# vicpc00/td-vc-gan

Measured on AMD Instinct MI355X. Metric: audio-seconds/sec (G+D train step, stage-1), higher is better.
Workload: dtype f32 (fp32 storage and accumulation everywhere; FiLM cond_var.2 forward and weight-grad as split-bf16 x6 products -- three exact bf16 pieces per operand, six piece products on the bf16 MFMA, fp32 accumulate: fp32-level accuracy; every other kernel exact-fp32 MFMA)

## Files before the change

td-vc-gan_amd/csrc/conv_api.hip:

```cpp
#include "../../include/tdvc.h"
#include "conv_common.h"
#include "conv_lean.h"
#include "conv_wgrad_lean.h"
#include "conv_small_group.h"
#include "api_util.h"

namespace tdvc {
template <int MODE> hipError_t launch_conv_gemm(GemmConvP, int, hipStream_t);
template <int MODE> hipError_t launch_conv_scalar(GemmConvP, int, hipStream_t);
template <int MODE> hipError_t launch_conv_wgrad(WgradP, int, int, hipStream_t);
template <int MODE> hipError_t launch_conv_wgrad_scalar(WgradP, int, long, float*, hipStream_t);
int wgrad_geometry(WgradP& p, int B, int* bpb_out);
bool wgrad_mfma_supported(int J);
hipError_t launch_slab_reduce(const float*, int, long, long, float*, int, long, hipStream_t, long n_w = -1, float* dbias = nullptr);
hipError_t launch_bias_grad(const Opnd&, int, int, int, float*, hipStream_t);
hipError_t fold_flush(hipStream_t st);
void fold_set_defer(int on);
void fold_reset(hipStream_t st);
}

namespace tdvc {


}

using namespace tdvc;

static inline bool al16(const void* p) { return (((uintptr_t)p) & 15) == 0; }
static inline bool ok_bs(const void* p, long bs) { return !p || (bs < (1L << 31)); }
static inline bool vec_ptr(const void* p, long bs) { return !p || (al16(p) && (bs & 3) == 0); }

static int lean_xfk(const tdvc_xform& x, float* slope, float* scale, const float** aux, long* aux_bs) {
  *scale = x.scale == 0.f ? 1.f : x.scale; *aux = x.aux; *aux_bs = x.aux_bs; *slope = x.slope;
  switch (x.kind) {
    case TDVC_XF_NONE: *slope = 1.f; *aux = nullptr; return LXF_ACT;
    case TDVC_XF_LRELU: *aux = nullptr; return (x.slope >= 0.f && x.slope <= 1.f) ? LXF_ACT : -1;
    case TDVC_XF_FILM_LRELU: return (x.slope >= 0.f && x.slope <= 1.f) ? LXF_FILM : -1;
    case TDVC_XF_MASK_LRELU: return LXF_MASK_LRELU;
    case TDVC_XF_MASK_TANH: return LXF_MASK_TANH;
    default: return -1;
  }
}

static bool lean_shape_ok(const tdvc_conv_desc* d) {
  return d->kind == TDVC_CONV && d->stride == 1 && d->groups == 1 && d->Tin == d->Tout && ((d->Tin & 3) == 0 || d->Tin <= 80);
}

namespace tdvc { int g_force_generic = 0; }
extern "C" void tdvc_set_force_generic(int on) { g_force_generic = on; }

static Xf to_xf(const tdvc_xform& x) {
  Xf r; r.kind = x.kind; r.slope = x.slope; r.scale = x.scale == 0.f ? 1.f : x.scale;
  r.aux = x.aux; r.aux_bs = x.aux_bs; return r;
}

static int check_desc(const tdvc_conv_desc* d) {
  if (!d) return tdvc_fail(TDVC_EINVAL, "null desc");
  if (d->B <= 0 || d->Cin <= 0 || d->Cout <= 0 || d->Tin <= 0 || d->Tout <= 0 || d->K <= 0 || d->stride <= 0 ||
      d->dilation <= 0 || d->groups <= 0 || d->pad < 0)
    return tdvc_fail(TDVC_EINVAL, "conv desc: non-positive dimension");
  if (d->Cin % d->groups || d->Cout % d->groups) return tdvc_fail(TDVC_EINVAL, "conv desc: channels not divisible by groups");
  if (d->stride > 1 && d->dilation != 1) return tdvc_fail(TDVC_EUNSUPPORTED, "strided conv with dilation");
  if (d->reflect && (d->stride != 1 || d->kind != TDVC_CONV)) return tdvc_fail(TDVC_EUNSUPPORTED, "reflect padding needs stride 1 conv");
  if (d->reflect && d->pad >= d->Tin) return tdvc_fail(TDVC_EINVAL, "reflect padding must be smaller than the input length");
  if (d->w_cin < 0 || d->w_cin_off < 0) return tdvc_fail(TDVC_EINVAL, "conv desc: negative weight channel window");
  if (d->w_cin > 0) {
    if (d->groups != 1 || d->kind != TDVC_CONV) return tdvc_fail(TDVC_EUNSUPPORTED, "weight channel window needs a plain conv with groups == 1");
    if (d->w_cin_off + d->Cin > d->w_cin) return tdvc_fail(TDVC_EINVAL, "conv desc: weight channel window out of range");
  }
  if (d->kind == TDVC_CONV) {
    long expect = ((long)d->Tin + 2L * d->pad - (long)d->dilation * (d->K - 1) - 1) / d->stride + 1;
    if (expect != d->Tout) return tdvc_fail(TDVC_EINVAL, "conv desc: Tout does not match conv arithmetic");
  } else if (d->kind == TDVC_CONV_TRANSPOSE) {
    if (d->stride < 2) return tdvc_fail(TDVC_EUNSUPPORTED, "transposed conv needs stride >= 2");
    long expect = ((long)d->Tin - 1) * d->stride - 2L * d->pad + (d->K - 1) + 1;
    if (d->Tout > expect + d->stride - 1 || d->Tout < expect) return tdvc_fail(TDVC_EINVAL, "conv desc: Tout does not match transposed conv arithmetic");
  } else return tdvc_fail(TDVC_EINVAL, "conv desc: unknown kind");
  return TDVC_OK;
}

static inline int ceil_div(int a, int b) { return (a + b - 1) / b; }

static bool small_group_ok(const tdvc_conv_desc* d) {
  return !g_force_generic && g_knob[2] == 0 && d->kind == TDVC_CONV && d->groups >= 16 && d->Cin == 4 * d->groups && d->Cout == 4 * d->groups &&
         d->dilation == 1 && !d->reflect && d->w_cin == 0 && d->stride >= 2 && d->stride <= 8 && d->K <= 48;
}
static void small_group_base(const tdvc_conv_desc* d, SmallGroupP& q) {
  q.B = d->B; q.G = d->groups; q.Tin = d->Tin; q.Tout = d->Tout; q.K = d->K; q.s = d->stride; q.pad = d->pad;
  q.in_scale = 1.f; q.out_scale = 1.f; q.dy_scale = 1.f;
}

static bool use_mfma(const GemmConvP& p) {
  if (g_force_generic) return false;
  if (p.R <= 2 && p.x.Cg == 1 && p.Cy_g <= 2) return false;
  return (long)p.Cred * p.J >= 7;
}

template <int MODE>
static int run_gemm(GemmConvP& p, int B, hipStream_t st) {
  hipError_t e = use_mfma(p) ? launch_conv_gemm<MODE>(p, B, st) : launch_conv_scalar<MODE>(p, B, st);
  return e == hipSuccess ? TDVC_OK : tdvc_fail(TDVC_ELAUNCH, hipGetErrorString(e));
}

static int dispatch_gemm(GemmConvP& p, int B, hipStream_t st) {
  switch (p.mode) {
    case MODE_DIRECT: return run_gemm<MODE_DIRECT>(p, B, st);
    case MODE_DOWN: return run_gemm<MODE_DOWN>(p, B, st);
    default: return run_gemm<MODE_UP>(p, B, st);
  }
}

extern "C" int tdvc_conv_fwd(const tdvc_conv_desc* d, const tdvc_conv_fwd_args* a, void* stream) {
  if (int rc = check_desc(d)) return rc;
  if (!a || !a->x || !a->w || !a->y) return tdvc_fail(TDVC_EINVAL, "conv_fwd: null pointer");
  const int Cin_g = d->Cin / d->groups, Cout_g = d->Cout / d->groups;
  if (small_group_ok(d) && a->x_xf.kind <= TDVC_XF_LRELU && !a->res && !a->add && !a->bias3) {
    SmallGroupP q = {};
    small_group_base(d, q);
    q.x = a->x; q.x_bs = a->x_bs; q.w = a->w; q.bias = a->bias; q.y = a->y; q.y_bs = a->y_bs;
    q.act_in = a->x_xf.kind == TDVC_XF_LRELU; q.slope_in = a->x_xf.slope; q.in_scale = a->x_xf.scale == 0.f ? 1.f : a->x_xf.scale;
    q.post = a->post_act; q.post_slope = a->post_slope; q.out_scale = a->out_scale == 0.f ? 1.f : a->out_scale;
    const hipError_t e = launch_small_group_fwd(q, (hipStream_t)stream);
    if (e == hipSuccess) return TDVC_OK;
    if (e != hipErrorNotSupported) return tdvc_fail(TDVC_ELAUNCH, hipGetErrorString(e));
  }
  if (!g_force_generic && lean_shape_ok(d) && (d->Cin & 3) == 0) {
    LeanP q = {};
    float slope, scale; const float* aux; long aux_bs;
    const int xfk = lean_xfk(a->x_xf, &slope, &scale, &aux, &aux_bs);
    const int cw = (d->w_cin > 0 ? d->w_cin : d->Cin) * d->K;
    const float* w = a->w + (long)d->w_cin_off * d->K;
    if (xfk >= 0 && (cw & 3) == 0 && al16(w) && ok_bs(a->x, a->x_bs) && ok_bs(a->y, a->y_bs) && ok_bs(a->res, a->res_bs) &&
        ok_bs(a->add, a->add_bs) && ok_bs(aux, aux_bs)) {
      q.x = a->x; q.w = w; q.y = a->y; q.bias = a->bias; q.bias3 = a->bias3; q.res = a->res; q.add = a->add; q.aux = aux;
      q.x_bs = (int)a->x_bs; q.y_bs = (int)a->y_bs; q.res_bs = (int)a->res_bs; q.add_bs = (int)a->add_bs; q.aux_bs = (int)aux_bs;
      q.T = d->Tin; q.Cin = d->Cin; q.Cout = d->Cout; q.Cw = cw; q.K = d->K; q.d = d->dilation; q.pad = d->pad; q.reflect = d->reflect;
      q.post = a->post_act; q.slope = slope; q.in_scale = scale; q.out_scale = a->out_scale == 0.f ? 1.f : a->out_scale;
      q.add_scale = 1.f; q.m_slope = a->post_slope;
      q.sbits = a->sign_bits; q.sb_bs = (int)a->sign_bits_bs;
      q.vec = ((d->Tin & 3) == 0 && vec_ptr(a->x, a->x_bs) && vec_ptr(a->y, a->y_bs) && vec_ptr(a->res, a->res_bs) &&
               vec_ptr(a->add, a->add_bs) && vec_ptr(aux, aux_bs)) ? 1 : 0;
      if (!q.vec && d->Tin > 80) goto generic_fwd;
      hipError_t e = launch_conv_lean(q, d->B, xfk, EPI_FWD, (hipStream_t)stream);
      if (e == hipSuccess) return TDVC_OK;
      if (e != hipErrorNotSupported) return tdvc_fail(TDVC_ELAUNCH, hipGetErrorString(e));
    }
  }
generic_fwd:
  if (a->sign_bits) return tdvc_fail(TDVC_EUNSUPPORTED, "conv_fwd: sign_bits needs a stride-1 conv with Tout % 32 == 0, Tout > 80 and 16-byte aligned operands");
  GemmConvP p = {};
  p.x.p = a->x; p.x.bs = a->x_bs; p.x.T = d->Tin; p.x.Cg = Cin_g; p.x.xf = to_xf(a->x_xf);
  p.w = a->w; p.K = d->K; p.s = d->stride; p.pad = d->pad; p.groups = d->groups;
  p.y = a->y; p.y_bs = a->y_bs; p.Ty = d->Tout; p.Cy_g = Cout_g;
  p.epi = EPI_FWD; p.bias = a->bias; p.bias3 = a->bias3; p.res = a->res; p.res_bs = a->res_bs;
  p.post = a->post_act; p.post_slope = a->post_slope; p.out_scale = a->out_scale == 0.f ? 1.f : a->out_scale;
  p.add = a->add; p.add_bs = a->add_bs; p.add_scale = 1.f;
  p.w_sg = (long)Cout_g * Cin_g * d->K;
  if (d->kind == TDVC_CONV) {
    p.w_sm = (long)Cin_g * d->K; p.w_sc = d->K;
    if (d->w_cin > 0) { p.w_sm = (long)d->w_cin * d->K; p.w += (long)d->w_cin_off * d->K; }
    p.R = Cout_g; p.N = d->Tout;
    if (d->stride == 1) { p.mode = MODE_DIRECT; p.Cred = Cin_g; p.J = d->K; p.d = d->dilation; p.reflect = d->reflect; }
    else { p.mode = MODE_DOWN; p.Cred = Cin_g * d->stride; p.J = ceil_div(d->K, d->stride); p.d = 1; }
  } else {
    p.w_sm = d->K; p.w_sc = (long)Cout_g * d->K;
    p.mode = MODE_UP; p.R = Cout_g * d->stride; p.Cred = Cin_g; p.J = ceil_div(d->K, d->stride); p.d = 1;
    p.N = (d->Tout - 1 + d->pad) / d->stride + 1;
  }
  return dispatch_gemm(p, d->B, (hipStream_t)stream);
}

extern "C" int tdvc_conv_dgrad(const tdvc_conv_desc* d, const tdvc_conv_dgrad_args* a, void* stream) {
  if (int rc = check_desc(d)) return rc;
  if (!a || !a->dy || !a->w || !a->dx) return tdvc_fail(TDVC_EINVAL, "conv_dgrad: null pointer");
  const int Cin_g = d->Cin / d->groups, Cout_g = d->Cout / d->groups;
  if (small_group_ok(d) && a->epilogue == TDVC_DG_PLAIN && !a->add &&
      (a->dy_xf.kind == TDVC_XF_NONE || (a->dy_xf.kind == TDVC_XF_MASK_LRELU && a->dy_xf.aux))) {
    SmallGroupP q = {};
    small_group_base(d, q);
    q.dy = a->dy; q.dy_bs = a->dy_bs; q.w = a->w; q.y = a->dx; q.y_bs = a->dx_bs;
    q.dy_scale = a->dy_xf.scale == 0.f ? 1.f : a->dy_xf.scale;
    if (a->dy_xf.kind == TDVC_XF_MASK_LRELU) { q.mask = a->dy_xf.aux; q.mask_bs = a->dy_xf.aux_bs; q.m_slope = a->dy_xf.slope; }
    const hipError_t e = launch_small_group_dgrad(q, (hipStream_t)stream);
    if (e == hipSuccess) return TDVC_OK;
    if (e != hipErrorNotSupported) return tdvc_fail(TDVC_ELAUNCH, hipGetErrorString(e));
  }
  if (!g_force_generic && a->wt && lean_shape_ok(d) && (d->Cout & 3) == 0 && (d->K - 1) * d->dilation - d->pad >= 0) {
    LeanP q = {};
    float slope, scale; const float* aux; long aux_bs;
    const int xfk = lean_xfk(a->dy_xf, &slope, &scale, &aux, &aux_bs);
    const int cw = d->Cout * d->K;
    const float* w = a->wt + (long)d->w_cin_off * cw;
    const int epi = a->epilogue == TDVC_DG_PLAIN ? EPI_PLAIN : (a->epilogue == TDVC_DG_MASK_LRELU ? EPI_MASK : EPI_FILM);
    if (xfk >= 0 && (cw & 3) == 0 && al16(w) && ok_bs(a->dy, a->dy_bs) && ok_bs(a->dx, a->dx_bs) && ok_bs(a->add, a->add_bs) &&
        ok_bs(aux, aux_bs) && ok_bs(a->x_in, a->x_in_bs) && ok_bs(a->gb, a->gb_bs) && ok_bs(a->dgb, a->dgb_bs) &&
        (epi == EPI_PLAIN || a->x_in || (epi == EPI_MASK && a->x_sign_bits)) && (epi != EPI_FILM || (a->gb && a->dgb))) {
      q.x = a->dy; q.w = w; q.y = a->dx; q.add = a->add; q.aux = aux; q.mx = a->x_in; q.gb = a->gb; q.dgb = a->dgb;
      q.x_bs = (int)a->dy_bs; q.y_bs = (int)a->dx_bs; q.add_bs = (int)a->add_bs; q.aux_bs = (int)aux_bs; q.mx_bs = (int)a->x_in_bs;
      q.gb_bs = (int)a->gb_bs; q.dgb_bs = (int)a->dgb_bs;
      q.T = d->Tin; q.Cin = d->Cout; q.Cout = d->Cin; q.Cw = cw; q.K = d->K; q.d = d->dilation;
      q.pad = (d->K - 1) * d->dilation - d->pad; q.flip = 1; q.mirror = d->reflect ? d->pad : 0;
      q.slope = slope; q.in_scale = scale; q.out_scale = 1.f; q.add_scale = a->add_scale; q.m_slope = a->slope;
      if (epi == EPI_MASK && a->x_sign_bits) { q.mbits = a->x_sign_bits; q.mb_bs = (int)a->x_sign_bits_bs; }
      q.vec = ((d->Tin & 3) == 0 && vec_ptr(a->dy, a->dy_bs) && vec_ptr(a->dx, a->dx_bs) && vec_ptr(a->add, a->add_bs) && vec_ptr(aux, aux_bs) &&
               vec_ptr(a->x_in, a->x_in_bs) && vec_ptr(a->gb, a->gb_bs) && vec_ptr(a->dgb, a->dgb_bs)) ? 1 : 0;
      if (!q.vec && d->Tin > 80) goto generic_dgrad;
      hipError_t e = launch_conv_lean(q, d->B, xfk, epi, (hipStream_t)stream);
      if (e == hipSuccess) return TDVC_OK;
      if (e != hipErrorNotSupported) return tdvc_fail(TDVC_ELAUNCH, hipGetErrorString(e));
      if (q.mbits && a->x_in) {
        q.mbits = nullptr;
        e = launch_conv_lean(q, d->B, xfk, epi, (hipStream_t)stream);
        if (e == hipSuccess) return TDVC_OK;
        if (e != hipErrorNotSupported) return tdvc_fail(TDVC_ELAUNCH, hipGetErrorString(e));
      }
    }
  }
generic_dgrad:
  if (a->epilogue == TDVC_DG_MASK_LRELU && !a->x_in && a->x_sign_bits)
    return tdvc_fail(TDVC_EUNSUPPORTED, "conv_dgrad: x_sign_bits without x_in needs a stride-1 conv with Tin % 32 == 0, Tin > 80 and 16-byte aligned operands");
  GemmConvP p = {};
  p.x.p = a->dy; p.x.bs = a->dy_bs; p.x.T = d->Tout; p.x.Cg = Cout_g; p.x.xf = to_xf(a->dy_xf);
  p.w = a->w; p.K = d->K; p.s = d->stride; p.groups = d->groups;
  p.y = a->dx; p.y_bs = a->dx_bs; p.Ty = d->Tin; p.Cy_g = Cin_g; p.N = d->Tin;
  p.add = a->add; p.add_bs = a->add_bs; p.add_scale = a->add_scale;
  p.w_sg = (long)Cout_g * Cin_g * d->K;
  switch (a->epilogue) {
    case TDVC_DG_PLAIN: p.epi = EPI_PLAIN; break;
    case TDVC_DG_MASK_LRELU:
      if (!a->x_in) return tdvc_fail(TDVC_EINVAL, "conv_dgrad: mask epilogue needs x_in");
      p.epi = EPI_MASK; p.mx = a->x_in; p.mx_bs = a->x_in_bs; p.m_slope = a->slope; break;
    case TDVC_DG_FILM:
      if (!a->x_in || !a->gb || !a->dgb) return tdvc_fail(TDVC_EINVAL, "conv_dgrad: FiLM epilogue needs x_in, gb, dgb");
      p.epi = EPI_FILM; p.mx = a->x_in; p.mx_bs = a->x_in_bs; p.m_slope = a->slope;
      p.gb = a->gb; p.gb_bs = a->gb_bs; p.dgb = a->dgb; p.dgb_bs = a->dgb_bs; break;
    default: return tdvc_fail(TDVC_EINVAL, "conv_dgrad: unknown epilogue");
  }
  if (d->kind == TDVC_CONV) {
    p.w_sm = d->K; p.w_sc = (long)Cin_g * d->K;
    if (d->w_cin > 0) { p.w_sc = (long)d->w_cin * d->K; p.w += (long)d->w_cin_off * d->K; }
    if (d->stride == 1) {
      p.mode = MODE_DIRECT; p.R = Cin_g; p.Cred = Cout_g; p.J = d->K; p.d = d->dilation; p.tap_flip = 1;
      p.pad = (d->K - 1) * d->dilation - d->pad;
      if (p.pad < 0) return tdvc_fail(TDVC_EUNSUPPORTED, "conv_dgrad: padding larger than the receptive field");
      p.mirror_pad = d->reflect ? d->pad : 0;
    } else {
      p.mode = MODE_UP; p.R = Cin_g * d->stride; p.Cred = Cout_g; p.J = ceil_div(d->K, d->stride); p.d = 1; p.pad = d->pad;
      p.N = (d->Tin - 1 + d->pad) / d->stride + 1;
    }
  } else {
    p.w_sm = (long)Cout_g * d->K; p.w_sc = d->K;
    p.mode = MODE_DOWN; p.R = Cin_g; p.Cred = Cout_g * d->stride; p.J = ceil_div(d->K, d->stride); p.d = 1; p.pad = d->pad;
  }
  return dispatch_gemm(p, d->B, (hipStream_t)stream);
}

static void fill_wgrad(const tdvc_conv_desc* d, const tdvc_conv_wgrad_args* a, WgradP& p) {
  const int Cin_g = d->Cin / d->groups, Cout_g = d->Cout / d->groups;
  p.groups = d->groups; p.K = d->K; p.s = d->stride; p.pad = d->pad;
  p.w_sg = (long)Cout_g * Cin_g * d->K;
  if (d->kind == TDVC_CONV) {
    if (a) { p.a.p = a->dy; p.a.bs = a->dy_bs; p.a.xf = to_xf(a->dy_xf); p.x.p = a->x; p.x.bs = a->x_bs; p.x.xf = to_xf(a->x_xf); }
    p.a.T = d->Tout; p.a.Cg = Cout_g; p.x.T = d->Tin; p.x.Cg = Cin_g;
    p.R = Cout_g; p.N = d->Tout; p.w_sm = (long)Cin_g * d->K; p.w_sc = d->K;
    if (d->stride == 1) { p.mode = MODE_DIRECT; p.Cred = Cin_g; p.J = d->K; p.d = d->dilation; p.reflect = d->reflect; }
    else { p.mode = MODE_DOWN; p.Cred = Cin_g * d->stride; p.J = ceil_div(d->K, d->stride); p.d = 1; }
  } else {
    if (a) { p.a.p = a->x; p.a.bs = a->x_bs; p.a.xf = to_xf(a->x_xf); p.x.p = a->dy; p.x.bs = a->dy_bs; p.x.xf = to_xf(a->dy_xf); }
    p.a.T = d->Tin; p.a.Cg = Cin_g; p.x.T = d->Tout; p.x.Cg = Cout_g;
    p.R = Cin_g; p.N = d->Tin; p.w_sm = (long)Cout_g * d->K; p.w_sc = d->K;
    p.mode = MODE_DOWN; p.Cred = Cout_g * d->stride; p.J = ceil_div(d->K, d->stride); p.d = 1;
  }
}

static bool wgrad_use_mfma(const WgradP& p) {
  if (g_force_generic) return false;
  if (p.R <= 2 && p.x.Cg == 1) return false;
  if (!wgrad_mfma_supported(p.J)) return false;
  return true;
}

static bool wgrad_lean_ok(const tdvc_conv_desc* d) {
  const bool wide = d->Cout >= 32 && d->Cin >= 32;
  return !g_force_generic && d->kind == TDVC_CONV && d->stride == 1 && d->groups == 1 && d->Tin == d->Tout &&
         (d->Tout > 128 || wide) && wgrad_lean_supported(d->K, d->dilation) && (d->K != 15 || d->Cout <= 16 || d->Cin <= 16);
}

namespace tdvc {
int wgrad_lean_nslab(int R, int Cin, int N, int K, int B);
bool wgrad_x6_ok(int R, int Cin, int T, int K, int dil, int pad, int reflect);
void wgrad_x6_plan(int R, int T, int B, int* ntiles, int* tpb, int* ngroups);
hipError_t launch_conv_wgrad_x6(const WgLeanP& q, int B, hipStream_t st);
}
static bool wgrad_x6_desc_ok(const tdvc_conv_desc* d) {
  return !g_force_generic && d->kind == TDVC_CONV && d->stride == 1 && d->groups == 1 && d->Tin == d->Tout && d->w_cin == 0 &&
         wgrad_x6_ok(d->Cout, d->Cin, d->Tout, d->K, d->dilation, d->pad, d->reflect);
}

extern "C" size_t tdvc_conv_wgrad_workspace(const tdvc_conv_desc* d) {
  if (check_desc(d)) return 0;
  size_t small = small_group_ok(d) ? small_group_wgrad_workspace(d->B, d->groups, d->K) : 0;
  if (wgrad_lean_ok(d)) {
    size_t lean = (size_t)wgrad_lean_nslab(d->Cout, d->Cin, d->Tout, d->K, d->B) * ((size_t)d->Cout * d->Cin * d->K + d->Cout) * sizeof(float);
    if (wgrad_x6_desc_ok(d)) {
      int nt, tpb, ng;
      wgrad_x6_plan(d->Cout, d->Tout, d->B, &nt, &tpb, &ng);
      const size_t x6 = (size_t)ng * ((size_t)d->Cout * d->Cin * d->K + d->Cout) * sizeof(float);
      if (x6 > lean) lean = x6;
    }
    return lean;
  }
  WgradP p = {};
  fill_wgrad(d, nullptr, p);
  if (!wgrad_use_mfma(p)) return small;
  int bpb;
  const int nslab = wgrad_geometry(p, d->B, &bpb);
  const long wsize = (long)d->groups * p.w_sg;
  const size_t gen = (size_t)nslab * (size_t)wsize * sizeof(float);
  return gen > small ? gen : small;
}

extern "C" int tdvc_conv_wgrad(const tdvc_conv_desc* d, const tdvc_conv_wgrad_args* a, void* stream) {
  if (int rc = check_desc(d)) return rc;
  if (!a || !a->x || !a->dy) return tdvc_fail(TDVC_EINVAL, "conv_wgrad: null pointer");
  hipStream_t st = (hipStream_t)stream;
  WgradP p = {};
  fill_wgrad(d, a, p);
  const long wsize = (long)d->groups * p.w_sg;
  hipError_t e = hipSuccess;
  bool done = false, bias_done = false;
  if (a->dw && small_group_ok(d) && a->x_xf.kind <= TDVC_XF_LRELU &&
      (a->dy_xf.kind == TDVC_XF_NONE || (a->dy_xf.kind == TDVC_XF_MASK_LRELU && a->dy_xf.aux))) {
    SmallGroupP q = {};
    small_group_base(d, q);
    q.x = a->x; q.x_bs = a->x_bs; q.dy = a->dy; q.dy_bs = a->dy_bs;
    q.act_in = a->x_xf.kind == TDVC_XF_LRELU; q.slope_in = a->x_xf.slope; q.in_scale = a->x_xf.scale == 0.f ? 1.f : a->x_xf.scale;
// ... 100 lines not shown
```

td-vc-gan_amd/csrc/conv_common.h:

```cpp
#pragma once
#include <hip/hip_runtime.h>
#include <stdint.h>
#include <mutex>

#define TDVC_BIG_LDS_ONCE(k)                                                                                         \
  do {                                                                                                               \
    static std::once_flag f_;                                                                                        \
    std::call_once(f_, [&] { hipFuncSetAttribute(reinterpret_cast<const void*>(k), hipFuncAttributeMaxDynamicSharedMemorySize, 160 * 1024); }); \
  } while (0)
namespace tdvc {
extern int g_trace_on;
extern int g_force_tile;
extern int g_force_generic;
extern int g_lds_cap;
extern int g_knob[8];
void trace_kernel(const void* fn);
}
#define TDVC_TRACE(k) do { if (tdvc::g_trace_on) tdvc::trace_kernel(reinterpret_cast<const void*>(k)); } while (0)

namespace tdvc {

enum { MODE_DIRECT = 0, MODE_DOWN = 1, MODE_UP = 2 };
enum { XF_NONE = 0, XF_LRELU = 1, XF_FILM_LRELU = 2, XF_MASK_LRELU = 3, XF_MASK_TANH = 4 };
enum { EPI_FWD = 0, EPI_MASK = 1, EPI_FILM = 2, EPI_PLAIN = 3 };
enum { POST_NONE = 0, POST_LRELU = 1, POST_TANH = 2 };

struct Xf {
  int kind; float slope; float scale;
  const float* aux; long aux_bs;
};

struct Opnd {
  const float* p; long bs; int T; int Cg; Xf xf;
};

struct GemmConvP {
  Opnd x;
  const float* w; long w_sg, w_sm, w_sc; int K; int tap_flip;
  int mode, s, d, pad, reflect, J;
  int R, Cred, Cc, N, groups, lo, span, XS, WS;
  int i0;
  int mirror_pad;
  int stage_rows;
  int chan_stage;
  int w_nat;
  int w_packed;
  float* y; long y_bs; int Ty; int Cy_g;
  int epi;
  const float* bias;
  const float* bias3;
  const float* res; long res_bs;
  int post; float post_slope; float out_scale;
  const float* add; long add_bs; float add_scale;
  const float* mx; long mx_bs; float m_slope;
  const float* gb; long gb_bs; float* dgb; long dgb_bs;
};

struct WgradP {
  Opnd a;
  Opnd x;
  int mode, s, d, pad, reflect, J, K;
  int R, Cred, N, groups, lo, span, NTc, XS, AS;
  int i0;
  int ntiles;
  float* slab; long slab_stride;
  long w_sg, w_sm, w_sc;
};

__device__ __forceinline__ float lrelu_f(float v, float s) { return v > 0.f ? v : v * s; }

__device__ __forceinline__ float apply_xf(const Xf& xf, float v, int b, int ch, int t, int T, int Ctot) {
  switch (xf.kind) {
    case XF_LRELU: v = lrelu_f(v, xf.slope); break;
    case XF_FILM_LRELU: {
      const float* g = xf.aux + (long)b * xf.aux_bs + (long)ch * T + t;
      v = lrelu_f(v * (1.f + g[0]) + g[(long)Ctot * T], xf.slope);
    } break;
    case XF_MASK_LRELU: {
      float a = xf.aux[(long)b * xf.aux_bs + (long)ch * T + t];
      v = a > 0.f ? v : v * xf.slope;
    } break;
    case XF_MASK_TANH: {
      float a = xf.aux[(long)b * xf.aux_bs + (long)ch * T + t];
      v = v * (1.f - a * a);
    } break;
    default: break;
  }
  return v * xf.scale;
}

__device__ __forceinline__ float fetch_opnd(const Opnd& o, int b, int ch, int q, int reflect, int Ctot) {
  if (reflect) {
    if (q < 0) q = -q;
    else if (q >= o.T) q = 2 * (o.T - 1) - q;
  }
  if (q < 0 || q >= o.T) return 0.f;
  float v = o.p[(long)b * o.bs + (long)ch * o.T + q];
  return apply_xf(o.xf, v, b, ch, q, o.T, Ctot);
}


typedef float f32x4_t __attribute__((ext_vector_type(4)));

__device__ __forceinline__ bool rows_align_ok(const Opnd& o, int q0, int span) {
  return (o.T & 3) == 0 && (o.bs & 3) == 0 && ((q0 | span) & 3) == 0 && (((uintptr_t)o.p) & 15) == 0 &&
         (o.xf.kind == XF_NONE || o.xf.kind == XF_LRELU || ((((uintptr_t)o.xf.aux) & 15) == 0 && (o.xf.aux_bs & 3) == 0));
}
__device__ __forceinline__ bool rows_fast_ok(const Opnd& o, int q0, int span) {
  return q0 >= 0 && q0 + span <= o.T && rows_align_ok(o, q0, span);
}

template <int NV>
struct RegTile { f32x4_t v[NV]; };

template <int NV>
__device__ __forceinline__ void tile_issue(RegTile<NV>& t, const float* base, int rowstride, int nvalid, int nrows, int span,
                                           int cvalid , int ebase, int tid,
                                           int vlo = 0, int vhi = 1 << 30 );
template <int NV>
__device__ __forceinline__ void tile_commit(const RegTile<NV>& t, const RegTile<NV>* a, const RegTile<NV>* c, const Xf& xf,
                                            float* dst, int XS, int nvalid, int nrows, int span, int ebase, int tid) {
  typedef float f32x2_t __attribute__((ext_vector_type(2)));
  const int nvec = span >> 2, total = nrows * nvec;
  const float inv = 1.0f / (float)nvec;
  const int kind = xf.kind;
  const float sl = xf.slope, sc = xf.scale;
#pragma unroll
  for (int i = 0; i < NV; ++i) {
    const int e = ebase + tid + i * 256;
    if (e >= total) continue;
    const int r = (int)(((float)e + 0.5f) * inv);
    const int vv = e - r * nvec;
    f32x4_t val = t.v[i];
    if (r < nvalid) {
      if (kind == XF_LRELU) {
#pragma unroll
        for (int q = 0; q < 4; ++q) val[q] = fmaxf(val[q], val[q] * sl);
      } else if (kind == XF_FILM_LRELU) {
#pragma unroll
        for (int q = 0; q < 4; ++q) { const float h = val[q] * (1.f + a->v[i][q]) + c->v[i][q]; val[q] = fmaxf(h, h * sl); }
      } else if (kind == XF_MASK_LRELU) {
#pragma unroll
        for (int q = 0; q < 4; ++q) val[q] = a->v[i][q] > 0.f ? val[q] : val[q] * sl;
      } else if (kind == XF_MASK_TANH) {
#pragma unroll
        for (int q = 0; q < 4; ++q) val[q] = val[q] * (1.f - a->v[i][q] * a->v[i][q]);
      }
      if (sc != 1.f) {
#pragma unroll
        for (int q = 0; q < 4; ++q) val[q] *= sc;
      }
    }
    f32x2_t* d2 = reinterpret_cast<f32x2_t*>(dst + r * XS + 4 * vv);
    d2[0] = (f32x2_t){val[0], val[1]};
    d2[1] = (f32x2_t){val[2], val[3]};
  }
}

typedef __amdgpu_buffer_rsrc_t srd_t;
typedef unsigned int u32x4_t __attribute__((ext_vector_type(4)));

__device__ __forceinline__ srd_t make_srd(const float* base, int bytes) {
  const uintptr_t a = reinterpret_cast<uintptr_t>(base);
  const unsigned lo = __builtin_amdgcn_readfirstlane((unsigned)(a & 0xffffffffu));
  const unsigned hi = __builtin_amdgcn_readfirstlane((unsigned)(a >> 32));
  const int nb = __builtin_amdgcn_readfirstlane(bytes > 0 ? bytes : 0);
  float* ub = reinterpret_cast<float*>(((uintptr_t)hi << 32) | lo);
  return __builtin_amdgcn_make_buffer_rsrc(ub, 0, nb, 0x00020000);
// ... 201 lines not shown
```

td-vc-gan_amd/csrc/misc_kernels.hip:

```cpp
#include "../../include/tdvc.h"
#include "api_util.h"
#include "conv_common.h"
#include <math.h>
#include <stdlib.h>
#include <string.h>

static thread_local char g_err[256] = "";
int tdvc_fail(int code, const char* msg) {
  snprintf(g_err, sizeof(g_err), "%s", msg ? msg : "");
  return code;
}
extern "C" const char* tdvc_last_error(void) { return g_err; }
extern "C" int tdvc_version(void) { return 200; }

#include <cxxabi.h>
#include <mutex>
#include <set>
#include <string>
namespace tdvc {
int g_trace_on = 0;
int g_force_tile = -1;
int g_lds_cap = 0;
int g_knob[8] = {0, 0, 0, 0, 0, 0, 0, 0};
static std::mutex g_trace_mu;
static std::set<std::string> g_trace_names;
void trace_kernel(const void* fn) {
  const char* mangled = hipKernelNameRefByPtr(fn, nullptr);
  std::string name;
  if (mangled) {
    int status = 0;
    char* dem = abi::__cxa_demangle(mangled, nullptr, nullptr, &status);
    name = (status == 0 && dem) ? dem : mangled;
    free(dem);
  } else {
    char buf[32]; snprintf(buf, sizeof(buf), "kernel@%p", fn); name = buf;
  }
  std::lock_guard<std::mutex> lk(g_trace_mu);
  g_trace_names.insert(name);
}
}
extern "C" void tdvc_debug_force_tile(int cfg) { tdvc::g_force_tile = cfg; }
extern "C" void tdvc_debug_lds_cap(int bytes) { tdvc::g_lds_cap = bytes; }
extern "C" void tdvc_debug_knob(int which, int value) { if (which >= 0 && which < 8) tdvc::g_knob[which] = value; }
namespace tdvc {
__global__ __launch_bounds__(256) void poison_lds_kernel(unsigned word, int nwords, unsigned* sink) {
  extern __shared__ __attribute__((aligned(16))) float smem[];
  unsigned* u = reinterpret_cast<unsigned*>(smem);
  for (int i = threadIdx.x; i < nwords; i += 256) u[i] = word;
  __syncthreads();
  unsigned acc = 0;
  for (int i = threadIdx.x; i < nwords; i += 256) acc ^= u[i];
  if (acc == 0x12345u && sink) sink[0] = acc;
}
}
extern "C" int tdvc_debug_poison_lds(uint32_t word, void* stream) {
  auto k = tdvc::poison_lds_kernel;
  TDVC_BIG_LDS_ONCE(k);
  hipLaunchKernelGGL(k, dim3(4096), dim3(256), 80 * 1024, (hipStream_t)stream, (unsigned)word, 80 * 1024 / 4, (unsigned*)nullptr);
  TDVC_CHECK_LAUNCH();
  return TDVC_OK;
}
namespace tdvc { __global__ void pmc_marker_kernel(int*) {} }
extern "C" int tdvc_debug_marker(void* stream) {
  hipLaunchKernelGGL(tdvc::pmc_marker_kernel, dim3(1), dim3(64), 0, (hipStream_t)stream, (int*)nullptr);
  TDVC_CHECK_LAUNCH();
  return TDVC_OK;
}
extern "C" void tdvc_debug_trace(int on) {
  std::lock_guard<std::mutex> lk(tdvc::g_trace_mu);
  if (on == 1) tdvc::g_trace_names.clear();
  tdvc::g_trace_on = on ? 1 : 0;
}
extern "C" size_t tdvc_debug_trace_dump(char* buf, size_t cap) {
  std::lock_guard<std::mutex> lk(tdvc::g_trace_mu);
  std::string all;
  for (const std::string& n : tdvc::g_trace_names) { all += n; all += '\n'; }
  if (buf && cap) { const size_t n = all.size() < cap - 1 ? all.size() : cap - 1; memcpy(buf, all.data(), n); buf[n] = 0; }
  return all.size() + 1;
}

namespace {

__device__ __forceinline__ float wave_sum(float v) {
#pragma unroll
  for (int o = 32; o > 0; o >>= 1) v += __shfl_xor(v, o);
  return v;
}

__device__ __forceinline__ float block_sum(float v, float* sh ) {
  v = wave_sum(v);
  __syncthreads();
  if ((threadIdx.x & 63) == 0) sh[threadIdx.x >> 6] = v;
  __syncthreads();
  float r = 0.f;
  const int nw = (blockDim.x + 63) >> 6;
  for (int i = 0; i < nw; ++i) r += sh[i];
  return r;
}

__global__ __launch_bounds__(256) void wn_fwd_kernel(const float* __restrict__ params, float* __restrict__ w,
                                                     const int64_t* row_voff, const int64_t* row_goff,
                                                     const int64_t* row_woff, const int32_t* row_len, int nrows,
                                                     float* __restrict__ wt, const int64_t* row_tbase,
                                                     const int64_t* row_tstride, const int32_t* row_k) {
  const int row = blockIdx.x * 4 + (threadIdx.x >> 6);
  if (row >= nrows) return;
  const int lane = threadIdx.x & 63;
  const float* v = params + row_voff[row];
  float* o = w + row_woff[row];
  const int n = row_len[row];
  float ss = 0.f;
  for (int i = lane; i < n; i += 64) { float t = v[i]; ss += t * t; }
  ss = wave_sum(ss);
  const float sc = params[row_goff[row]] / sqrtf(ss);
  const int K = wt ? row_k[row] : 0;
  if (K > 0) {
    float* tb = wt + row_tbase[row];
    const long ts = row_tstride[row];
    for (int i = lane; i < n; i += 64) {
      const float val = v[i] * sc;
      o[i] = val;
      const int ci = i / K;
      tb[(long)ci * ts + (i - ci * K)] = val;
    }
  } else {
    for (int i = lane; i < n; i += 64) o[i] = v[i] * sc;
  }
}

__global__ __launch_bounds__(256) void wn_bwd_kernel(const float* __restrict__ params, const float* __restrict__ dw,
                                                     float* __restrict__ grads, const int64_t* row_voff,
                                                     const int64_t* row_goff, const int64_t* row_woff,
                                                     const int32_t* row_len, int nrows, int accumulate) {
  const int row = blockIdx.x * 4 + (threadIdx.x >> 6);
  if (row >= nrows) return;
  const int lane = threadIdx.x & 63;
  const float* v = params + row_voff[row];
  const float* d = dw + row_woff[row];
  float* dv = grads + row_voff[row];
  const int n = row_len[row];
  float ss = 0.f, dot = 0.f;
  for (int i = lane; i < n; i += 64) { float t = v[i]; ss += t * t; dot += t * d[i]; }
  ss = wave_sum(ss); dot = wave_sum(dot);
  const float nrm = sqrtf(ss), g = params[row_goff[row]];
  const float a = g / nrm, bcoef = g * dot / (nrm * ss);
  for (int i = lane; i < n; i += 64) {
    const float t = a * d[i] - bcoef * v[i];
    dv[i] = accumulate ? dv[i] + t : t;
  }
  if (lane == 0) {
    float* dg = grads + row_goff[row];
    const float t = dot / nrm;
    dg[0] = accumulate ? dg[0] + t : t;
  }
}

__global__ __launch_bounds__(256) void adamw_kernel(float* __restrict__ p, const float* __restrict__ g, float* __restrict__ m,
                                                    float* __restrict__ v, long n, float lr, float b1, float b2, float eps,
                                                    float wd, float bc1, float bc2_sqrt, float gscale, const int32_t* step_ptr,
                                                    const float* gscale_dev) {
  if (gscale_dev) gscale *= gscale_dev[0];
  if (step_ptr) {
    const float st = (float)step_ptr[0];
    bc1 = 1.f - powf(b1, st); bc2_sqrt = sqrtf(1.f - powf(b2, st));
  }
  for (long i = (long)blockIdx.x * 256 + threadIdx.x; i < n; i += (long)gridDim.x * 256) {
    const float gr = g[i] * gscale;
    float pv = p[i] * (1.f - lr * wd);
    const float mv = b1 * m[i] + (1.f - b1) * gr;
    const float vv = b2 * v[i] + (1.f - b2) * gr * gr;
    const float denom = sqrtf(vv) / bc2_sqrt + eps;
    pv -= (lr / bc1) * (mv / denom);
    p[i] = pv; m[i] = mv; v[i] = vv;
  }
}

__global__ __launch_bounds__(256) void l2norm_fwd_kernel(const float* x, float* y, float* inv, int C, int T, float eps) {
  const int t = blockIdx.x * 256 + threadIdx.x, b = blockIdx.y;
  if (t >= T) return;
  const float* xb = x + (long)b * C * T + t;
  float ss = 0.f;
  for (int c = 0; c < C; ++c) { float v = xb[(long)c * T]; ss += v * v; }
  const float r = 1.f / fmaxf(sqrtf(ss), eps);
  inv[(long)b * T + t] = r;
  float* yb = y + (long)b * C * T + t;
  for (int c = 0; c < C; ++c) yb[(long)c * T] = xb[(long)c * T] * r;
}

__global__ __launch_bounds__(256) void l2norm_bwd_kernel(const float* y, const float* inv, const float* dy, float* dx, int C, int T) {
  const int t = blockIdx.x * 256 + threadIdx.x, b = blockIdx.y;
  if (t >= T) return;
  const long o = (long)b * C * T + t;
  float dot = 0.f;
  for (int c = 0; c < C; ++c) dot += dy[o + (long)c * T] * y[o + (long)c * T];
  const float r = inv[(long)b * T + t];
  for (int c = 0; c < C; ++c) dx[o + (long)c * T] = (dy[o + (long)c * T] - y[o + (long)c * T] * dot) * r;
// ... 817 lines not shown
```

Measured before the change: 300.0.

## Add specialized MFMA kernels for stride-4 grouped convs with 4-in/16-out channels

Adds a dedicated forward and data-grad kernel for grouped convolutions with 4 input and 16 output channels per group, stride 4 and K between 41 and 43. Each wave keeps the group's weights in registers, stages input tiles through a per-wave LDS slab, and prefetches the next tile's loads while issuing fp32 16x16x4 MFMAs. Work is spread over a fixed wave budget with a persistent per-wave item loop. The aim is to replace the generic GEMM/scalar path for these layers, at the cost of new specialized code and a new knob slot.

```diff
diff --git a/td-vc-gan_amd/csrc/conv_api.hip b/td-vc-gan_amd/csrc/conv_api.hip
--- a/td-vc-gan_amd/csrc/conv_api.hip
+++ b/td-vc-gan_amd/csrc/conv_api.hip
@@ -3,6 +3,7 @@
 #include "conv_lean.h"
 #include "conv_wgrad_lean.h"
 #include "conv_small_group.h"
+#include "conv_group16.h"
 #include "api_util.h"
 
 namespace tdvc {
@@ -90,6 +91,21 @@
   q.in_scale = 1.f; q.out_scale = 1.f; q.dy_scale = 1.f;
 }
 
+static bool group16_ok(const tdvc_conv_desc* d) {
+  return !g_force_generic && g_knob[8] == 0 && d->kind == TDVC_CONV && d->dilation == 1 && !d->reflect && d->w_cin == 0 &&
+         group16_shape_ok(d->Cin, d->Cout, d->groups, d->K, d->stride);
+}
+static void group16_base(const tdvc_conv_desc* d, Group16P& q) {
+  q.B = d->B; q.G = d->groups; q.Tin = d->Tin; q.Tout = d->Tout; q.K = d->K; q.pad = d->pad;
+  q.out_scale = 1.f; q.dy_scale = 1.f;
+}
+static bool unit_xf(const tdvc_xform& x) { return x.kind == TDVC_XF_NONE && (x.scale == 0.f || x.scale == 1.f); }
+static bool group16_dy_ok(const tdvc_xform& x) { return x.kind == TDVC_XF_NONE || (x.kind == TDVC_XF_MASK_LRELU && x.aux); }
+static void group16_dy(const tdvc_xform& x, Group16P& q) {
+  q.dy_scale = x.scale == 0.f ? 1.f : x.scale;
+  if (x.kind == TDVC_XF_MASK_LRELU) { q.mask = x.aux; q.mask_bs = x.aux_bs; q.m_slope = x.slope; }
+}
+
 static bool use_mfma(const GemmConvP& p) {
   if (g_force_generic) return false;
   if (p.R <= 2 && p.x.Cg == 1 && p.Cy_g <= 2) return false;
@@ -121,6 +137,15 @@
     q.act_in = a->x_xf.kind == TDVC_XF_LRELU; q.slope_in = a->x_xf.slope; q.in_scale = a->x_xf.scale == 0.f ? 1.f : a->x_xf.scale;
     q.post = a->post_act; q.post_slope = a->post_slope; q.out_scale = a->out_scale == 0.f ? 1.f : a->out_scale;
     const hipError_t e = launch_small_group_fwd(q, (hipStream_t)stream);
+    if (e == hipSuccess) return TDVC_OK;
+    if (e != hipErrorNotSupported) return tdvc_fail(TDVC_ELAUNCH, hipGetErrorString(e));
+  }
+  if (group16_ok(d) && unit_xf(a->x_xf) && !a->res && !a->add && !a->bias3 && !a->sign_bits) {
+    Group16P q = {};
+    group16_base(d, q);
+    q.x = a->x; q.x_bs = a->x_bs; q.w = a->w; q.bias = a->bias; q.y = a->y; q.y_bs = a->y_bs;
+    q.post = a->post_act; q.post_slope = a->post_slope; q.out_scale = a->out_scale == 0.f ? 1.f : a->out_scale;
+    const hipError_t e = launch_group16_fwd(q, (hipStream_t)stream);
     if (e == hipSuccess) return TDVC_OK;
     if (e != hipErrorNotSupported) return tdvc_fail(TDVC_ELAUNCH, hipGetErrorString(e));
   }
@@ -182,6 +207,15 @@
     q.dy_scale = a->dy_xf.scale == 0.f ? 1.f : a->dy_xf.scale;
     if (a->dy_xf.kind == TDVC_XF_MASK_LRELU) { q.mask = a->dy_xf.aux; q.mask_bs = a->dy_xf.aux_bs; q.m_slope = a->dy_xf.slope; }
     const hipError_t e = launch_small_group_dgrad(q, (hipStream_t)stream);
+    if (e == hipSuccess) return TDVC_OK;
+    if (e != hipErrorNotSupported) return tdvc_fail(TDVC_ELAUNCH, hipGetErrorString(e));
+  }
+  if (group16_ok(d) && a->epilogue == TDVC_DG_PLAIN && !a->add && group16_dy_ok(a->dy_xf)) {
+    Group16P q = {};
+    group16_base(d, q);
+    q.dy = a->dy; q.dy_bs = a->dy_bs; q.w = a->w; q.y = a->dx; q.y_bs = a->dx_bs;
+    group16_dy(a->dy_xf, q);
+    const hipError_t e = launch_group16_dgrad(q, (hipStream_t)stream);
     if (e == hipSuccess) return TDVC_OK;
     if (e != hipErrorNotSupported) return tdvc_fail(TDVC_ELAUNCH, hipGetErrorString(e));
   }
diff --git a/td-vc-gan_amd/csrc/conv_common.h b/td-vc-gan_amd/csrc/conv_common.h
--- a/td-vc-gan_amd/csrc/conv_common.h
+++ b/td-vc-gan_amd/csrc/conv_common.h
@@ -13,7 +13,7 @@
 extern int g_force_tile;
 extern int g_force_generic;
 extern int g_lds_cap;
-extern int g_knob[8];
+extern int g_knob[16];
 void trace_kernel(const void* fn);
 }
 #define TDVC_TRACE(k) do { if (tdvc::g_trace_on) tdvc::trace_kernel(reinterpret_cast<const void*>(k)); } while (0)
diff --git a/td-vc-gan_amd/csrc/conv_group16.h b/td-vc-gan_amd/csrc/conv_group16.h
--- /dev/null
+++ b/td-vc-gan_amd/csrc/conv_group16.h
@@ -0,0 +1,25 @@
+#pragma once
+#include <hip/hip_runtime.h>
+
+namespace tdvc {
+
+struct Group16P {
+  const float* x; long x_bs;
+  const float* w;
+  const float* bias;
+  const float* dy; long dy_bs;
+  const float* mask; long mask_bs;
+  float* y; long y_bs;
+  int B, G, Tin, Tout, K, pad;
+  int M;
+  int ntile;
+  int per_wave;
+  int post; float post_slope, out_scale, dy_scale, m_slope;
+  int vec;
+};
+
+bool group16_shape_ok(int Cin, int Cout, int groups, int K, int stride);
+hipError_t launch_group16_fwd(Group16P p, hipStream_t st);
+hipError_t launch_group16_dgrad(Group16P p, hipStream_t st);
+
+}
diff --git a/td-vc-gan_amd/csrc/conv_group16.hip b/td-vc-gan_amd/csrc/conv_group16.hip
--- /dev/null
+++ b/td-vc-gan_amd/csrc/conv_group16.hip
@@ -0,0 +1,226 @@
+#include "conv_common.h"
+#include "conv_group16.h"
+
+namespace tdvc {
+
+typedef float f32x4 __attribute__((ext_vector_type(4)));
+
+constexpr int G16_J = 11;
+constexpr int G16_NT = 64;
+constexpr int G16_S = 80;
+constexpr int G16_WAVES = 2048;
+
+static __device__ __forceinline__ float g16_load(srd_t rs, int elem, bool ok) {
+  return __builtin_bit_cast(float, __builtin_amdgcn_raw_buffer_load_b32(rs, ok ? elem * 4 : 0x7f000000, 0, 0));
+}
+
+static __device__ __forceinline__ void g16_wave_sync() {
+  __builtin_amdgcn_fence(__ATOMIC_RELEASE, "wavefront"); __builtin_amdgcn_wave_barrier(); __builtin_amdgcn_fence(__ATOMIC_ACQUIRE, "wavefront");
+}
+
+static __device__ __forceinline__ float g16_post(float v, int post, float slope) {
+  if (post == POST_LRELU) return v > 0.f ? v : v * slope;
+  if (post == POST_TANH) return tanhf(v);
+  return v;
+}
+
+__global__ __launch_bounds__(256) void group16_fwd_kernel(const Group16P p) {
+  __shared__ __attribute__((aligned(16))) float sm[4][4 * 4 * G16_S];
+  const int lane = threadIdx.x & 63, wave = threadIdx.x >> 6;
+  const int t16 = lane & 15, kq = lane >> 4;
+  const long nitems = (long)p.G * p.B * p.ntile;
+  const long i0 = ((long)blockIdx.x * 4 + wave) * p.per_wave;
+  const long i1 = min(nitems, i0 + (long)p.per_wave);
+  if (i0 >= i1) return;
+  float* xs = sm[wave];
+  float wr[4 * G16_J];
+  float xv[4][5];
+  int gcur = -1;
+  auto issue = [&](long it) {
+    const int tile = (int)(it % p.ntile); const long gb = it / p.ntile;
+    const int b = (int)(gb % p.B), g = (int)(gb / p.B);
+    const int q0 = tile * G16_NT * 4 - p.pad;
+    const srd_t rs = make_srd(p.x + (long)b * p.x_bs + (long)g * 4 * p.Tin, 4 * p.Tin * 4);
+#pragma unroll
+    for (int ci = 0; ci < 4; ++ci)
+#pragma unroll
+      for (int i = 0; i < 5; ++i) {
+        const int q = q0 + lane + 64 * i;
+        xv[ci][i] = g16_load(rs, ci * p.Tin + q, q >= 0 && q < p.Tin);
+      }
+  };
+  issue(i0);
+  for (long it = i0; it < i1; ++it) {
+    const int tile = (int)(it % p.ntile); const long gb = it / p.ntile;
+    const int b = (int)(gb % p.B), g = (int)(gb / p.B);
+    if (g != gcur) {
+      gcur = g;
+      const srd_t ws = make_srd(p.w + (long)g * 64 * p.K, 64 * p.K * 4);
+#pragma unroll
+      for (int ci = 0; ci < 4; ++ci)
+#pragma unroll
+        for (int j = 0; j < G16_J; ++j) {
+          const int k = 4 * j + kq;
+          wr[ci * G16_J + j] = g16_load(ws, t16 * 4 * p.K + ci * p.K + k, k < p.K);
+        }
+    }
+    g16_wave_sync();
+#pragma unroll
+    for (int ci = 0; ci < 4; ++ci)
+#pragma unroll
+      for (int i = 0; i < 5; ++i) {
+        const int e = lane + 64 * i;
+        xs[ci * 4 * G16_S + (e & 3) * G16_S + (e >> 2)] = xv[ci][i];
+      }
+    g16_wave_sync();
+    if (it + 1 < i1) issue(it + 1);
+    f32x4 acc[4];
+#pragma unroll
+    for (int m = 0; m < 4; ++m) acc[m] = (f32x4){0.f, 0.f, 0.f, 0.f};
+#pragma unroll
+    for (int j = 0; j < G16_J; ++j)
+#pragma unroll
+      for (int ci = 0; ci < 4; ++ci) {
+        const float bw = wr[ci * G16_J + j];
+        const float* xr = xs + ci * 4 * G16_S + kq * G16_S + t16 + j;
+#pragma unroll
+        for (int m = 0; m < 4; ++m) acc[m] = __builtin_amdgcn_mfma_f32_16x16x4f32(xr[16 * m], bw, acc[m], 0, 0, 0);
+      }
+    const int ch = g * 16 + t16;
+    const float bv = p.bias ? p.bias[ch] : 0.f;
+    float* yr = p.y + (long)b * p.y_bs + (long)ch * p.Tout;
+#pragma unroll
+    for (int m = 0; m < 4; ++m) {
+      const int t = tile * G16_NT + 16 * m + 4 * kq;
+      f32x4 v;
+#pragma unroll
+      for (int r = 0; r < 4; ++r) v[r] = g16_post(acc[m][r] + bv, p.post, p.post_slope) * p.out_scale;
+      if (p.vec && t + 3 < p.Tout) *reinterpret_cast<f32x4*>(yr + t) = v;
+      else {
+#pragma unroll
+        for (int r = 0; r < 4; ++r)
+          if (t + r < p.Tout) yr[t + r] = v[r];
+      }
+    }
+  }
+}
+
+__global__ __launch_bounds__(256) void group16_dgrad_kernel(const Group16P p) {
+  __shared__ __attribute__((aligned(16))) float sm[4][16 * G16_S];
+  const int lane = threadIdx.x & 63, wave = threadIdx.x >> 6;
+  const int t16 = lane & 15, kq = lane >> 4;
+  const long nitems = (long)p.G * p.B * p.ntile;
+  const long i0 = ((long)blockIdx.x * 4 + wave) * p.per_wave;
+  const long i1 = min(nitems, i0 + (long)p.per_wave);
+  if (i0 >= i1) return;
+  float* ds = sm[wave];
+  float wr[4 * G16_J];
+  float dv[20], mv[20] = {};
+  int gcur = -1;
+  auto issue = [&](long it) {
+    const int tile = (int)(it % p.ntile); const long gb = it / p.ntile;
+    const int b = (int)(gb % p.B), g = (int)(gb / p.B);
+    const int tb = tile * G16_NT - (G16_J - 1);
+    const srd_t rs = make_srd(p.dy + (long)b * p.dy_bs + (long)g * 16 * p.Tout, 16 * p.Tout * 4);
+#pragma unroll
+    for (int i = 0; i < 20; ++i) {
+      const int e = lane + 64 * i, co = e / G16_S, u = e - co * G16_S, t = tb + u;
+      dv[i] = g16_load(rs, co * p.Tout + t, u < G16_NT + G16_J - 1 && t >= 0 && t < p.Tout);
+    }
+    if (p.mask) {
+      const srd_t ms = make_srd(p.mask + (long)b * p.mask_bs + (long)g * 16 * p.Tout, 16 * p.Tout * 4);
+#pragma unroll
+      for (int i = 0; i < 20; ++i) {
+        const int e = lane + 64 * i, co = e / G16_S, u = e - co * G16_S, t = tb + u;
+        mv[i] = g16_load(ms, co * p.Tout + t, u < G16_NT + G16_J - 1 && t >= 0 && t < p.Tout);
+      }
+    }
+  };
+  issue(i0);
+  for (long it = i0; it < i1; ++it) {
+    const int tile = (int)(it % p.ntile); const long gb = it / p.ntile;
+    const int b = (int)(gb % p.B), g = (int)(gb / p.B);
+    if (g != gcur) {
+      gcur = g;
+      const srd_t ws = make_srd(p.w + (long)g * 64 * p.K, 64 * p.K * 4);
+      const int ci = t16 >> 2, r = t16 & 3;
+#pragma unroll
+      for (int c4 = 0; c4 < 4; ++c4)
+#pragma unroll
+        for (int j = 0; j < G16_J; ++j) {
+          const int k = 4 * j + r;
+          wr[c4 * G16_J + j] = g16_load(ws, (4 * c4 + kq) * 4 * p.K + ci * p.K + k, k < p.K);
+        }
+    }
+    g16_wave_sync();
+#pragma unroll
+    for (int i = 0; i < 20; ++i) {
+      const float v = (!p.mask || mv[i] > 0.f) ? dv[i] : dv[i] * p.m_slope;
+      ds[lane + 64 * i] = v * p.dy_scale;
+    }
+    g16_wave_sync();
+    if (it + 1 < i1) issue(it + 1);
+    f32x4 acc[4];
+#pragma unroll
+    for (int m = 0; m < 4; ++m) acc[m] = (f32x4){0.f, 0.f, 0.f, 0.f};
+#pragma unroll
+    for (int jj = 0; jj < G16_J; ++jj)
+#pragma unroll
+      for (int c4 = 0; c4 < 4; ++c4) {
+        const int j = G16_J - 1 - jj;
+        const float aw = wr[c4 * G16_J + j];
+        const float* dr = ds + (4 * c4 + kq) * G16_S + t16 + G16_J - 1 - j;
+#pragma unroll
+        for (int m = 0; m < 4; ++m) acc[m] = __builtin_amdgcn_mfma_f32_16x16x4f32(aw, dr[16 * m], acc[m], 0, 0, 0);
+      }
+    float* dxr = p.y + (long)b * p.y_bs + (long)(g * 4 + kq) * p.Tin;
+#pragma unroll
+    for (int m = 0; m < 4; ++m) {
+      const int q = 4 * (tile * G16_NT + 16 * m + t16) - p.pad;
+      const f32x4 v = acc[m];
+      if (p.vec && q >= 0 && q + 3 < p.Tin) *reinterpret_cast<f32x4*>(dxr + q) = v;
+      else {
+#pragma unroll
+        for (int r = 0; r < 4; ++r)
+          if (q + r >= 0 && q + r < p.Tin) dxr[q + r] = v[r];
+      }
+    }
+  }
+}
+
+bool group16_shape_ok(int Cin, int Cout, int groups, int K, int stride) {
+  return Cin == 4 * groups && Cout == 16 * groups && stride == 4 && K >= 4 * (G16_J - 1) + 1 && K <= 4 * G16_J - 1;
+}
+
+static bool g16_sizes_ok(const Group16P& p) {
+  return (long)16 * p.Tout * 4 < (1L << 31) && (long)4 * p.Tin * 4 < (1L << 31) && p.Tout > 0 && p.Tin > 0 && p.pad >= 0;
+}
+
+static inline int g16_per_wave(long nitems) { return (int)((nitems + G16_WAVES - 1) / G16_WAVES); }
+
+hipError_t launch_group16_fwd(Group16P p, hipStream_t st) {
+  if (!group16_shape_ok(4 * p.G, 16 * p.G, p.G, p.K, 4) || !g16_sizes_ok(p)) return hipErrorNotSupported;
+  p.ntile = (p.Tout + G16_NT - 1) / G16_NT;
+  const long nitems = (long)p.G * p.B * p.ntile;
+  p.per_wave = g16_per_wave(nitems);
+  const long waves = (nitems + p.per_wave - 1) / p.per_wave;
+  p.vec = (p.Tout & 3) == 0 && (p.y_bs & 3) == 0 && (((uintptr_t)p.y) & 15) == 0;
+  TDVC_TRACE(group16_fwd_kernel);
+  hipLaunchKernelGGL(group16_fwd_kernel, dim3((unsigned)((waves + 3) / 4)), dim3(256), 0, st, p);
+  return hipGetLastError();
+}
+
+hipError_t launch_group16_dgrad(Group16P p, hipStream_t st) {
+  if (!group16_shape_ok(4 * p.G, 16 * p.G, p.G, p.K, 4) || !g16_sizes_ok(p)) return hipErrorNotSupported;
+  p.M = (p.Tin - 1 + p.pad) / 4 + 1;
+  p.ntile = (p.M + G16_NT - 1) / G16_NT;
+  const long nitems = (long)p.G * p.B * p.ntile;
+  p.per_wave = g16_per_wave(nitems);
+  const long waves = (nitems + p.per_wave - 1) / p.per_wave;
+  p.vec = (p.pad & 3) == 0 && (p.Tin & 3) == 0 && (p.y_bs & 3) == 0 && (((uintptr_t)p.y) & 15) == 0;
+  TDVC_TRACE(group16_dgrad_kernel);
+  hipLaunchKernelGGL(group16_dgrad_kernel, dim3((unsigned)((waves + 3) / 4)), dim3(256), 0, st, p);
+  return hipGetLastError();
+}
+
+}
diff --git a/td-vc-gan_amd/csrc/misc_kernels.hip b/td-vc-gan_amd/csrc/misc_kernels.hip
--- a/td-vc-gan_amd/csrc/misc_kernels.hip
+++ b/td-vc-gan_amd/csrc/misc_kernels.hip
@@ -21,7 +21,7 @@
 int g_trace_on = 0;
 int g_force_tile = -1;
 int g_lds_cap = 0;
-int g_knob[8] = {0, 0, 0, 0, 0, 0, 0, 0};
+int g_knob[16] = {0};
 static std::mutex g_trace_mu;
 static std::set<std::string> g_trace_names;
 void trace_kernel(const void* fn) {
@@ -41,7 +41,7 @@
 }
 extern "C" void tdvc_debug_force_tile(int cfg) { tdvc::g_force_tile = cfg; }
 extern "C" void tdvc_debug_lds_cap(int bytes) { tdvc::g_lds_cap = bytes; }
-extern "C" void tdvc_debug_knob(int which, int value) { if (which >= 0 && which < 8) tdvc::g_knob[which] = value; }
+extern "C" void tdvc_debug_knob(int which, int value) { if (which >= 0 && which < 16) tdvc::g_knob[which] = value; }
 namespace tdvc {
 __global__ __launch_bounds__(256) void poison_lds_kernel(unsigned word, int nwords, unsigned* sink) {
   extern __shared__ __attribute__((aligned(16))) float smem[];
```

Result: faster. 306.2 (median of 6 runs) (+2.1%).
